# astra-vision/PaSCo

Hardware: AMD Instinct MI355X
Metric: scenes/sec (256x256x32, ~10% occ) PaSCo MIMO-3 (higher is better)
Workload: dtype f32 (conv products as 3 x f16 split MFMA, fp32 accumulate)

## Files before the change

pasco_amd/csrc/conv_grid.hip:

```cpp
#include <math.h>
#include <stdlib.h>

#include "conv_h2_common.h"

constexpr int GR_WROWS = 264;
constexpr int GR_PIECES = GR_WROWS / 8;
constexpr int GR_ROUNDS = (GR_PIECES + 7) / 8;
constexpr int GR_WIN = GR_WROWS * 128;
constexpr int GR_BST = 128 * 128;
constexpr int GR_OFF_WIN = 2 * GR_BST;
constexpr int GR_OFF_ZERO = GR_OFF_WIN + 2 * GR_WIN;
constexpr int GR_OFF_MISC = GR_OFF_ZERO + 128;
constexpr int GR_LDS = GR_OFF_MISC + 64;

template <bool EMIT>
__global__ void __launch_bounds__(512, 2) k_conv_grid(ConvArgsH a) {
  constexpr int WN = 2, TM = 2, TN = 2;
  constexpr int NT = 512;
  constexpr int BM = 256, BN = 128;
  constexpr int NMH = TM * TN * 3;
  constexpr int NRH = (TM + TN) * 2;
  __shared__ __attribute__((aligned(128))) char lds[GR_LDS];

  int tile = blockIdx.x;
  if (PH_ABLATE(a, 0x200)) tile = ((int)blockIdx.x & 7) * ((int)gridDim.x >> 3) + ((int)blockIdx.x >> 3);
  if (tile >= a.n_row_tiles * a.n_col_tiles) return;
  const int row_tile = tile / a.n_col_tiles;
  const int col_tile = tile - row_tile * a.n_col_tiles;
  const int64_t m0 = (int64_t)row_tile * BM;
  const int n0 = col_tile * BN;

  const int tid = threadIdx.x;
  const int lane = tid & 63;
  const int wave = __builtin_amdgcn_readfirstlane(tid >> 6);
  const int wm = wave / WN, wn = wave % WN;
  const int h = lane >> 5;
  const int l31 = lane & 31;

  const int GX = a.gdim[1], GY = a.gdim[2], GZ = a.gdim[3];
  const int kx = a.gker[0], ky = a.gker[1], kz = a.gker[2];
  const int hx = kx >> 1, hy = ky >> 1, hz = kz >> 1;
  const int ngroups = kx * kz;
  const int cout = a.cout;
  const int nchunks = a.cpad >> 5;
  const uint32_t rsb = 4u * (uint32_t)a.cpad;
  const int slice = (int)blockIdx.y;

  f32x16 acc[TM][TN];
#pragma unroll
  for (int i = 0; i < TM; ++i)
#pragma unroll
    for (int j = 0; j < TN; ++j)
#pragma unroll
      for (int r = 0; r < 16; ++r) acc[i][j][r] = 0.f;

  unsigned *gmask = reinterpret_cast<unsigned *>(lds + GR_OFF_MISC);
  if (tid < 2) gmask[tid] = 0u;
  if (tid < 32) reinterpret_cast<float *>(lds + GR_OFF_ZERO)[tid] = 0.f;
  __syncthreads();
  {
    const int r = tid & 255;
    const int64_t s = m0 + r;
    const bool ok = s < a.n_out;
    const int t = (int)((ok ? s : 0) / GY);
    const int x = t % GX, zz = (t / GX) % GZ;
    for (int g = tid >> 8; g < ngroups; g += 2) {
      const int ix = g % kx, iz = g / kx;
      const bool v = ok && (unsigned)(x + ix - hx) < (unsigned)GX && (unsigned)(zz + iz - hz) < (unsigned)GZ;
      if (__ballot(v) != 0ull && lane == 0) atomicOr(&gmask[g >> 5], 1u << (g & 31));
    }
  }
  __syncthreads();
  const unsigned long long gm =
      (unsigned long long)(unsigned)__builtin_amdgcn_readfirstlane(gmask[0]) |
      ((unsigned long long)(unsigned)__builtin_amdgcn_readfirstlane(gmask[1]) << 32);
  const int nvalid = __builtin_popcountll(gm);
  const int total_units = nvalid * nchunks;
  int nsl = a.ksplit;
  if (a.grid_upw > 0) {
    nsl = (total_units + (a.grid_upw >> 1)) / a.grid_upw;
    nsl = nsl < 1 ? 1 : (nsl > a.ksplit ? a.ksplit : nsl);
  }
  const int nunits = (slice < nsl && slice < total_units) ? (total_units - slice + nsl - 1) / nsl : 0;
  const int nstages = nunits * ky;

  if (nstages > 0) {
    struct Unit {
      int n, vi, g, c;
    };
    const int kq = nsl / nchunks, kr = nsl - kq * nchunks;
    const int inv_kx = 65536 / kx + 1;
    auto first_unit = [&]() {
      Unit u;
      u.n = 0;
      u.vi = slice / nchunks;
      u.c = slice - u.vi * nchunks;
      unsigned long long m = gm;
      for (int q = 0; q < u.vi; ++q) m &= m - 1;
      u.g = __builtin_ctzll(m);
      return u;
    };
    auto next_unit = [&](const Unit &p) {
      Unit u;
      u.n = p.n + 1;
      u.c = p.c + kr;
      u.vi = p.vi + kq;
      if (u.c >= nchunks) {
        u.c -= nchunks;
        ++u.vi;
      }
      unsigned long long m = gm & ~((2ull << p.g) - 1ull);
      int g = p.g;
      for (int q = p.vi; q < u.vi; ++q) {
        g = __builtin_ctzll(m);
        m &= m - 1;
      }
      u.g = g;
      return u;
    };

    const int l_j = tid & 7;
    const int l_r = tid >> 3;
    const uint32_t sj16 = (uint32_t)((l_j ^ ((l_r >> 1) & 7)) << 4);
    const uint64_t w_base = (uint64_t)reinterpret_cast<uintptr_t>(a.w_split) + sj16;
    uint32_t boff[2];
#pragma unroll
    for (int q = 0; q < 2; ++q) {
      int n = n0 + l_r + q * 64;
      n = n < cout ? n : cout - 1;
      boff[q] = (uint32_t)n * rsb;
    }
    const int64_t wslab = (int64_t)cout * rsb;
    const uint64_t in_base = (uint64_t)reinterpret_cast<uintptr_t>(a.in_split);
    const int wl_r = lane >> 3;
    const int n_last = (int)(a.n_in - 1);
    const uint32_t wdst0 = (uint32_t)(wave * 1024);
    const uint32_t bdst0 = (uint32_t)(wave * 1024);

    auto fire_b = [&](uint64_t src, char *bbuf, int q) {
      if (PH_ABLATE(a, 2)) return;
      char *dst = bbuf + bdst0 + q * 8192;
      __builtin_amdgcn_global_load_lds((const __attribute__((address_space(1))) void *)(uintptr_t)(src + boff[q]),
                                       (__attribute__((address_space(3))) void *)dst, 16, 0, 0);
    };
    auto fire_win = [&](int first, uint32_t coff, uint32_t wbuf, int round) {
      if (PH_ABLATE(a, 1)) return;
      const int R = round * 64 + wave * 8 + wl_r;
      int site = first + R;
      site = site < 0 ? 0 : (site > n_last ? n_last : site);
      const uint64_t src = in_base + (uint64_t)(uint32_t)site * rsb + coff + (uint32_t)((l_j ^ ((R >> 1) & 7)) << 4);
      char *dst = lds + wbuf + round * 8192 + wdst0;
      __builtin_amdgcn_global_load_lds((const __attribute__((address_space(1))) void *)(uintptr_t)src,
                                       (__attribute__((address_space(3))) void *)dst, 16, 0, 0);
    };
    struct WinSrc {
      int first;
      uint32_t coff, wbuf;
    };
    auto win_of = [&](const Unit &u) {
      const int iz = (u.g * inv_kx) >> 16, ix = u.g - iz * kx;
      WinSrc w;
      w.first = (int)m0 + (ix - hx) * GY + (iz - hz) * GX * GY - hy;
      w.coff = (uint32_t)u.c << 7;
      w.wbuf = (uint32_t)(GR_OFF_WIN + (u.n & 1) * GR_WIN);
      return w;
    };

    int ay[TM], ax[TM], az[TM];
    bool aok[TM];
    uint32_t rbase[TM];
#pragma unroll
    for (int i = 0; i < TM; ++i) {
      rbase[i] = (uint32_t)(wm * 64 + i * 32 + l31);
      const int64_t s = m0 + rbase[i];
      aok[i] = s < a.n_out;
      const int sc = aok[i] ? (int)s : 0;
      const int t = sc / GY;
      ay[i] = sc - t * GY;
      ax[i] = t % GX;
      az[i] = (t / GX) % GZ;
    }
    const uint32_t hq = (uint32_t)h << 4;
    struct ASet {
      uint32_t row[TM], sw[TM];
    };
    bool gv[TM];
    uint32_t cwb = 0;
    auto unit_valid = [&](const Unit &u) {
      const int iz = (u.g * inv_kx) >> 16, ix = u.g - iz * kx;
      cwb = (uint32_t)(GR_OFF_WIN + (u.n & 1) * GR_WIN);
#pragma unroll
      for (int i = 0; i < TM; ++i)
        gv[i] = aok[i] && (unsigned)(ax[i] + ix - hx) < (unsigned)GX && (unsigned)(az[i] + iz - hz) < (unsigned)GZ;
    };
    auto a_set = [&](int iy, ASet &s) {
#pragma unroll
      for (int i = 0; i < TM; ++i) {
        const uint32_t R = rbase[i] + (uint32_t)iy;
        const bool v = gv[i] && (unsigned)(ay[i] + iy - hy) < (unsigned)GY;
        s.row[i] = v ? cwb + R * 128u : (uint32_t)GR_OFF_ZERO;
        s.sw[i] = ((R >> 1) & 7u) << 4;
      }
    };

    const int sw = (l31 >> 1) & 7;
    uint32_t xo[2][2];
#pragma unroll
    for (int ks = 0; ks < 2; ++ks)
#pragma unroll
      for (int part = 0; part < 2; ++part) xo[ks][part] = (uint32_t)(((part * 4 + ks * 2 + h) ^ sw) << 4);
    const uint32_t brow = (uint32_t)((wn * TN * 32 + l31) * 128);
    struct Frag {
      f16x8 ah[2][TM], al[2][TM], bh[2][TN], bl[2][TN];
    };
    Frag f;
    ASet aset;
    auto read_one = [&](const char *bbuf, int ks, int r) {
      if (PH_ABLATE(a, 8)) return;
      if (r < 2 * TM) {
        const int i = r >> 1, part = r & 1;
        const uint32_t o = aset.row[i] + ((((uint32_t)(part * 4 + ks * 2) << 4) | hq) ^ aset.sw[i]);
        if (part == 0) f.ah[ks][i] = *reinterpret_cast<const f16x8 *>(lds + o);
        else f.al[ks][i] = *reinterpret_cast<const f16x8 *>(lds + o);
      } else {
        const int j = (r - 2 * TM) >> 1;
        if (((r - 2 * TM) & 1) == 0) f.bh[ks][j] = *reinterpret_cast<const f16x8 *>(bbuf + brow + j * 4096 + xo[ks][0]);
        else f.bl[ks][j] = *reinterpret_cast<const f16x8 *>(bbuf + brow + j * 4096 + xo[ks][1]);
      }
    };
    auto mfma_one = [&](int ks, int m) {
      if (PH_ABLATE(a, 4)) return;
      const int ij = m % (TM * TN), p = m / (TM * TN);
      const int i = ij / TN, j = ij % TN;
      if (p == 0) acc[i][j] = __builtin_amdgcn_mfma_f32_32x32x16_f16(f.bh[ks][j], f.al[ks][i], acc[i][j], 0, 0, 0);
      else if (p == 1) acc[i][j] = __builtin_amdgcn_mfma_f32_32x32x16_f16(f.bl[ks][j], f.ah[ks][i], acc[i][j], 0, 0, 0);
      else acc[i][j] = __builtin_amdgcn_mfma_f32_32x32x16_f16(f.bh[ks][j], f.ah[ks][i], acc[i][j], 0, 0, 0);
    };

    Unit cu = first_unit(), du = cu;
    int ciy = 0, diy = 0;
    bool nu_ok = nunits > 1;
    Unit nu = nu_ok ? next_unit(cu) : cu;
    WinSrc nw = win_of(nu);
    uint64_t wsrc = w_base + (uint64_t)((int64_t)(ky * du.g) * wslab) + ((uint32_t)du.c << 7);
    auto d_step = [&]() {
      if (du.n == nunits - 1 && diy == ky - 1) return;
      if (++diy == ky) {
        diy = 0;
        du = next_unit(du);
        wsrc = w_base + (uint64_t)((int64_t)(ky * du.g) * wslab) + ((uint32_t)du.c << 7);
      } else {
        wsrc += (uint64_t)wslab;
      }
    };
    const int rps = (GR_ROUNDS + ky - 2) / (ky - 1);

    char *b0 = lds, *b1 = lds + GR_BST;
    {
      const WinSrc w0 = win_of(cu);
      for (int q = 0; q < GR_ROUNDS; ++q)
        if (q * 8 + wave < GR_PIECES) fire_win(w0.first, w0.coff, w0.wbuf, q);
    }
    fire_b(wsrc, b0, 0);
    fire_b(wsrc, b0, 1);
    d_step();
    fire_b(wsrc, b1, 0);
    fire_b(wsrc, b1, 1);
    d_step();
    unit_valid(cu);
    a_set(0, aset);
    asm volatile("s_waitcnt vmcnt(0) lgkmcnt(0)" ::: "memory");
    __builtin_amdgcn_s_barrier();
#pragma unroll
    for (int r = 0; r < NRH; ++r) read_one(b0, 0, r);
    asm volatile("s_waitcnt lgkmcnt(0)" ::: "memory");

    auto half_a = [&](const char *cur) {
#pragma unroll
      for (int g = 0; g < NRH; ++g) {
        read_one(cur, 1, g);
        __builtin_amdgcn_sched_barrier(0);
#pragma unroll
        for (int m = g * NMH / NRH; m < (g + 1) * NMH / NRH; ++m) mfma_one(0, m);
        __builtin_amdgcn_sched_barrier(0);
      }
    };
    auto half_b = [&](char *cur, const char *nxt) {
      int wq = (nu_ok && ciy < ky - 1) ? ciy * rps : GR_ROUNDS;
      const int wq_end = wq + rps;
      const WinSrc w = nw;
      if (!(cu.n == nunits - 1 && ciy == ky - 1)) {
        if (++ciy == ky) {
          ciy = 0;
          cu = nu;
          nu_ok = cu.n + 1 < nunits;
          if (nu_ok) {
            nu = next_unit(cu);
            nw = win_of(nu);
          }
          unit_valid(cu);
        }
      }
      if (!PH_ABLATE(a, 64)) a_set(ciy, aset);
#pragma unroll
      for (int g = 0; g < NRH; ++g) {
        if (g < 2) fire_b(wsrc, cur, g);
        if (g >= 2 && g < 5) {
          if (wq < wq_end && wq * 8 + wave < GR_PIECES) fire_win(w.first, w.coff, w.wbuf, wq);
          ++wq;
        }
        read_one(nxt, 0, g);
        if (g == 5) d_step();
        __builtin_amdgcn_sched_barrier(0);
#pragma unroll
        for (int m = g * NMH / NRH; m < (g + 1) * NMH / NRH; ++m) mfma_one(1, m);
        __builtin_amdgcn_sched_barrier(0);
      }
    };
#define GRID_MIDDLE()                                                            \
  do {                                                                           \
    if (PH_ABLATE(a, 16)) asm volatile("s_waitcnt lgkmcnt(0)" ::: "memory");     \
    else asm volatile("s_waitcnt vmcnt(0) lgkmcnt(0)" ::: "memory");             \
    if (!PH_ABLATE(a, 32)) __builtin_amdgcn_s_barrier();                         \
  } while (0)
    for (int s = 0; s < nstages; s += 2) {
      half_a(b0);
      GRID_MIDDLE();
      half_b(b0, b1);
      asm volatile("s_waitcnt lgkmcnt(0)" ::: "memory");
      if (s + 1 >= nstages) break;
      half_a(b1);
      GRID_MIDDLE();
      half_b(b1, b0);
      asm volatile("s_waitcnt lgkmcnt(0)" ::: "memory");
    }
    asm volatile("s_waitcnt vmcnt(0)" ::: "memory");
#undef GRID_MIDDLE
  }

  h2_store_tile<TM, TN, EMIT>(a, acc, m0, n0, wm, wn, h, l31);
}

#ifdef PH_DEV
static int g_grid_ablate = 0;
extern "C" void ph_conv_grid_set_ablate(int mask) { g_grid_ablate = mask; }
#else
constexpr int g_grid_ablate = 0;
#endif

static double grid_groups(const int *gd, const int *gk) {
  double zavg = 0.0;
  for (int z = 0; z < gd[3]; ++z)
    for (int iz = 0; iz < gk[2]; ++iz) zavg += (z + iz - gk[2] / 2 >= 0 && z + iz - gk[2] / 2 < gd[3]) ? 1.0 : 0.0;
  return gk[0] * zavg / gd[3];
}

int ph_conv_grid_try(const ConvArgsH &a_in, hipStream_t st) {
  const int *gd = a_in.gdim, *gk = a_in.gker;
  if (gd[0] <= 0 || a_in.tile_k != nullptr || a_in.win_gather || (a_in.cpad & 31) || a_in.cout % 128 != 0 || a_in.in_split == nullptr ||
      a_in.axis_table != nullptr)
    return -1;
  if (a_in.route & PH_ROUTE_GRID_NEVER) return -1;
  const int kx = gk[0], ky = gk[1], kz = gk[2];
  if (ky < 3 || ky > 7 || !(kx & 1) || !(ky & 1) || !(kz & 1) || kx * kz > 64 || kx * ky * kz != a_in.kvol) return -1;
  const int64_t sites = (int64_t)gd[0] * gd[1] * gd[2] * gd[3];
  if (sites != a_in.n_out || sites != a_in.n_in || gd[2] < 1) return -1;
  ConvArgsH a = a_in;
  a.n_row_tiles = (int)((a.n_out + 255) / 256);
  a.n_col_tiles = a.cout / 128;
  const int64_t tiles = (int64_t)a.n_row_tiles * a.n_col_tiles;
  const int nchunks = a.cpad >> 5;
  const double units = grid_groups(gd, gk) * nchunks;
  const double stage_us = 1.0, fixed_us = 8.0;
  int best = 1;
  double best_us = 1e30;
  for (int ks = 1; ks <= 12; ++ks) {
    if (ks > 1 && (a.tail_ws == nullptr || a.tail_ws_bytes < (int64_t)ks * a.n_out * a.cout * 4)) break;
    if (ks > 1 && units / ks < 2.0) break;
    const double rounds = (double)((tiles * ks + 255) / 256);
    double us = rounds * (ceil(units / ks) * ky * stage_us + fixed_us);
    if (ks > 1) us += (double)ks * (double)a.n_out * a.cout * 4.0 / 3.0e6 + 5.0;
    if (us < best_us) best_us = us, best = ks;
  }
  if (const char *e = PH_DEV_ENV("PASCO_GRID_KS")) {
    const int ks = atoi(e);
    if (ks >= 1 && (ks == 1 || (a.tail_ws != nullptr && a.tail_ws_bytes >= (int64_t)ks * a.n_out * a.cout * 4))) best = ks;
  }
  a.grid_upw = 0;
  if (best > 1 && tiles * best <= 256) {
    const int upw = (int)(units / best + 0.5) > 0 ? (int)(units / best + 0.5) : 1;
    int zmax = 0;
    for (int z = 0; z < gd[3]; ++z) {
      int c = 0;
      for (int iz = 0; iz < kz; ++iz) c += (z + iz - kz / 2 >= 0 && z + iz - kz / 2 < gd[3]) ? 1 : 0;
      zmax = c > zmax ? c : zmax;
    }
    const int zreach = zmax + 1 < kz ? zmax + 1 : kz;
    int ksmax = (kx * zreach * nchunks + upw / 2) / upw;
    ksmax = ksmax > 12 ? 12 : ksmax;
    while (ksmax > best && a.tail_ws_bytes < (int64_t)ksmax * a.n_out * a.cout * 4) --ksmax;
    const char *e = PH_DEV_ENV("PASCO_GRID_UPW");
    if (e == nullptr || atoi(e) != 0) {
      if (ksmax > best) best = ksmax;
      a.grid_upw = upw;
    }
  }
  a.ksplit = best;
  a.partial = best > 1 ? (float *)a.tail_ws : nullptr;
  a.win_stats = nullptr;
  a.ablate = g_grid_ablate;
  const int grid = (int)((tiles + 7) / 8) * 8;
  const bool emit = a.out_split != nullptr && a.ksplit == 1;
  if (emit) hipLaunchKernelGGL((k_conv_grid<true>), dim3(grid, 1), dim3(512), 0, st, a);
  else hipLaunchKernelGGL((k_conv_grid<false>), dim3(grid, a.ksplit), dim3(512), 0, st, a);
  PH_LAUNCH_CHECK();
  if (a.ksplit > 1) {
    if (int rc = ph_launch_splitk_epilogue(a, st)) return rc;
  }
  ph_record_cfg(2, 256, 128, 32, a.ksplit, emit ? 1 : 0, 8, 8);
  return 0;
}
```

pasco_amd/me/backend.py:

```python
from __future__ import annotations

import contextlib
import ctypes as C
import os
import threading
from typing import Dict, Optional

import torch

from .._clib import _raw_stream, bind

_HERE = os.path.dirname(os.path.abspath(__file__))
HIP_LIB_PATH = os.path.join(os.path.dirname(_HERE), "csrc", "libpascohip.so")

ACT_NONE, ACT_RELU, ACT_LEAKY = 0, 1, 2
ABI_VERSION = 5


class StatusError(RuntimeError):

    def __init__(self, bits: int, message: str):
        super().__init__(message)
        self.bits = bits

# ... 383 lines not shown
                        raise ValueError(f"conv: {name} has {t.numel()} entries, expected {cout}")
            d.out_split, d.osp_scale, d.osp_shift, d.osp_act = _ptr(out_split), _ptr(osc), _ptr(osh), int(oact)
        d.in_, d.weight, d.nbr, d.out = (None if x.is_meta else _ptr(x)), _ptr(weight), _ptr(nbr), _ptr(out)
        d.n_in, d.n_out, d.cin, d.cout, d.kvol = x.shape[0], n_out, cin, cout, kvol
        d.pro_act, d.epi_act, d.res_act, d.epi_slope = pro_act, epi_act, res_act, float(slope)
        for name, t, c in (("pro_scale", pro_scale, cin), ("pro_shift", pro_shift, cin),
                           ("bias", bias, cout), ("epi_scale", epi_scale, cout),
                           ("epi_shift", epi_shift, cout), ("epi2_scale", epi2_scale, cout),
                           ("epi2_shift", epi2_shift, cout)):
            if t is not None:
                self._chk(t, torch.float32, name)
                if t.numel() != c:
                    raise ValueError(f"conv: {name} has {t.numel()} entries, expected {c}")
            setattr(d, name, _ptr(t))
        if residual is not None:
            self._chk(residual, torch.float32, "residual")
            if tuple(residual.shape) != (n_out, cout):
                raise ValueError("conv: residual shape mismatch")
        d.residual = _ptr(residual)
        if axis is not None:
            tab, acoords, lo = axis
            self._chk(tab, torch.float32, "axis table")
            self._chk(acoords, torch.int32, "axis coords")
            if tab.dim() != 3 or tab.shape[0] != 3 or tab.shape[2] != cout or tuple(acoords.shape) != (n_out, 4):
                raise ValueError("conv: axis = (table [3, T, cout], coords [n_out, 4], lo)")
            if self.device_type == "cuda" and (split is None or len(split) != 2):
                raise ValueError("conv: the axis-table residual is served by the pre-split (mode 2) path")
            d.axis_table, d.axis_coords, d.axis_lo, d.axis_rows = _ptr(tab), _ptr(acoords), int(lo), int(tab.shape[1])
        if split is not None:
            if len(split) == 2:
                w_split, unscale = split
                if in_split is None:
                    in_split = self.split_rows(x, pro_scale=pro_scale, pro_shift=pro_shift, pro_act=pro_act, slope=slope)
                elif not x.is_meta and (pro_scale is not None or pro_shift is not None or pro_act != ACT_NONE) and \
                        not in_split_has_prologue:
                    raise ValueError("conv: in_split given together with a prologue - pass in_split_has_prologue=True if "
                                     "the operand was built with split_rows(x, pro_scale=..., pro_shift=..., pro_act=...), "
                                     "else drop in_split")
                cpad = (cin + 31) // 32 * 32
                if in_split.dtype != torch.float16 or in_split.numel() != x.shape[0] * 2 * cpad:
                    raise ValueError("conv: in_split does not match the input rows")
                if w_split.numel() != kvol * cout * 2 * cpad:
                    raise ValueError("conv: w_split does not match the kernel")
                d.mma_mode, d.in_split, d.w_split = 2, _ptr(in_split), _ptr(w_split)
                if grid is not None and nbr is not None:
                    gd, gk = grid
                    if len(gd) != 4 or len(gk) != 3 or gd[0] * gd[1] * gd[2] * gd[3] != n_out or x.shape[0] != n_out or \
                            gk[0] * gk[1] * gk[2] != kvol or any(k % 2 == 0 for k in gk):
                        raise ValueError("conv: grid = ((B, X, Y, Z), (kx, ky, kz)) must describe the whole map (odd kernel sizes)")
                    for q in range(4):
                        d.grid_dims[q] = int(gd[q])
                    for q in range(3):
                        d.grid_kernel[q] = int(gk[q])
                if rowlist is not None and nbr is not None:
                    d.rl_in, d.rl_out, d.rl_tile_k = _ptr(rowlist["in"]), _ptr(rowlist["out"]), _ptr(rowlist["tile_k"])
                    d.rl_rows, d.rl_tiles = int(rowlist["in"].numel()), int(rowlist["tile_k"].numel())
                if win is not None and kvol == 27 and nbr is not None:
                    d.win_rows, d.win_cnt, d.win_slots, d.win_stats = (_ptr(win["rows"]), _ptr(win["cnt"]),
                                                                       _ptr(win["slots"]), _ptr(win["stats"]))
                    if 32 < cout <= 64 and self._serves_cuda:
                        d.w_frag = _ptr(self.weight_fragments(w_split, kvol, cout, cpad))
            else:
                w_hi, w_lo, unscale = split
                d.mma_mode, d.w_f16_hi, d.w_f16_lo = 1, _ptr(w_hi), _ptr(w_lo)
            d.split_exp2 = SPLIT_ACT_EXP2
            d.w_unscale = float(unscale) * 2.0 ** (-SPLIT_ACT_EXP2)
            d.status = self.status_ptr(dev) if status is None else status.data_ptr()
            if kvol > 1 or n_out * cout <= (1 << 23):
                need = 12 * n_out * cout * 4 if n_out * cout <= (1 << 23) else 512 * 128 * 128 * 4
                key = ("splitk",) + self._stream_key(dev)
                sk = self._ws.get(key)
                if sk is None or sk.numel() < need:
                    sk = torch.empty(need, dtype=torch.uint8, device=dev)
                    self._ws[key] = sk
                d.splitk_ws, d.splitk_ws_bytes = _ptr(sk), sk.numel()
        if exact_if is not None:
            if split is not None:
                raise ValueError("conv: exact_if guards an exact fp32 launch (no split)")
            d.exact_if = exact_if.data_ptr()
        rc = self.fn["conv_fwd"](C.byref(d), self.stream(dev))
        self._check(rc, "conv_fwd")
        return (out, out_split) if emit else out

    @staticmethod
    def grid_offsets(kernel_size) -> list:
        kx, ky, kz = (int(k) for k in kernel_size)
        return [(x, y, z) for z in range(-(kz // 2), kz // 2 + 1) for x in range(-(kx // 2), kx // 2 + 1)
                for y in range(-(ky // 2), ky // 2 + 1)]

    def conv_last_config(self) -> dict:
        buf = (_i32 * 8)()
        self._check(self.fn["conv_last_config"](C.cast(buf, _vp)), "conv_last_config")
        names = ("mma_mode", "bm", "bn", "kc", "ksplit", "emit", "kernel", "waves")
        return dict(zip(names, [int(v) for v in buf]))

    def status_word(self, device) -> torch.Tensor:
        return self._status_pair(device)[0:1]

    def status_ptr(self, device) -> int:
        pinned = getattr(self._tls, "status_pin", None)
        if pinned is not None:
            return pinned.data_ptr()
        idx = device.index
        if idx is None and device.type == "cuda":
            idx = torch.cuda.current_device()
        k = (device.type, idx, _raw_stream(idx) if device.type == "cuda" else 0)
# ... 66 lines not shown
        w = weight.detach().float()
        if w.dim() == 2:
            w = w[None]
        if exponent is not None:
            e = int(exponent)
        else:
            wmax = float(w.abs().max())
            e = 0 if wmax == 0.0 else 13 - int(torch.frexp(torch.tensor(wmax))[1])
        scaled = (w * float(2.0 ** e)).transpose(1, 2).contiguous()
        hi = scaled.to(torch.float16)
        lo = (scaled - hi.float()).to(torch.float16)
        return hi.contiguous(), lo.contiguous(), float(2.0 ** (-e))

    def split_rows(self, x: torch.Tensor, *, pro_scale=None, pro_shift=None, pro_act=ACT_NONE, slope=0.01,
                   out: Optional[torch.Tensor] = None, exp2: Optional[int] = None,
                   status: Optional[torch.Tensor] = None) -> torch.Tensor:
        exp2 = SPLIT_ACT_EXP2 if exp2 is None else int(exp2)
        self._chk(x, torch.float32, "in")
        n, c = x.shape
        if c % 8 != 0:
            raise ValueError("split_rows: needs c % 8 == 0")
        cpad = (c + 31) // 32 * 32
        if out is None:
            out = torch.empty((n, cpad // 32, 2, 32), dtype=torch.float16, device=x.device)
        for name, t in (("pro_scale", pro_scale), ("pro_shift", pro_shift)):
            if t is not None:
                self._chk(t, torch.float32, name)
                if t.numel() != c:
                    raise ValueError(f"split_rows: {name} has {t.numel()} entries, expected {c}")
        rc = self.fn["split_rows"](_ptr(x), n, c, _ptr(pro_scale), _ptr(pro_shift), pro_act, float(slope), exp2, _ptr(out),
                                   self.status_ptr(x.device) if status is None else status.data_ptr(), self.stream(x.device))
        self._check(rc, "split_rows")
        return out

    def split_weight_rows(self, weight: torch.Tensor, exponent=None):
        w = weight.detach().float()
        if w.dim() == 2:
            w = w[None]
        if exponent is not None:
            e = int(exponent)
        else:
            wmax = float(w.abs().max())
            e = 0 if wmax == 0.0 else 13 - int(torch.frexp(torch.tensor(wmax))[1])
        k, cin, cout = w.shape
        rows = (w * float(2.0 ** e)).transpose(1, 2).contiguous().view(k * cout, cin)
        return self.split_rows(rows, exp2=0), float(2.0 ** (-e))

    @staticmethod
    def weight_fragments(w_split: torch.Tensor, kvol: int, cout: int, cpad: int) -> torch.Tensor:
        hit = getattr(w_split, "_ph_wfrag", None)
        if hit is not None and hit[0] == (kvol, cout, cpad):
            return hit[1]
        g = cpad // 32
        ws = w_split.view(kvol, cout, g, 2, 2, 2, 8)
        rows = torch.arange(64, device=w_split.device).clamp_(max=cout - 1)
        ws = ws.index_select(1, rows).view(kvol, 2, 32, g, 2, 2, 2, 8)
        frag = ws.permute(0, 3, 5, 1, 4, 6, 2, 7).contiguous()
        frag = frag.view(kvol, 2 * g, 2, 2, 64, 8)
        try:
            w_split._ph_wfrag = ((kvol, cout, cpad), frag)
        except AttributeError:
            pass
        return frag

    def split_capable(self) -> bool:
        return self.device_type == "cuda" or self.checker_split

    def split_supported(self, cin: int, cout: int) -> bool:
        return self.split_capable() and cin % 8 == 0 and cout % 4 == 0

    def maxpool_fwd(self, x: torch.Tensor, nbr: torch.Tensor) -> torch.Tensor:
        self._chk(x, torch.float32, "in")
        self._chk(nbr, torch.int32, "nbr")
        kvol, n_out = nbr.shape
        out = torch.empty((n_out, x.shape[1]), dtype=torch.float32, device=x.device)
        rc = self.fn["maxpool_fwd"](_ptr(x), x.shape[1], _ptr(nbr), kvol, n_out, _ptr(out),
                                    self.stream(x.device))
        self._check(rc, "maxpool_fwd")
        return out

    def mask_compact(self, mask: torch.Tensor) -> torch.Tensor:
        if mask.dtype == torch.bool:
            mask = mask.view(torch.uint8)
        self._chk(mask, torch.uint8, "mask")
        n = mask.shape[0]
        dev = mask.device
        buf = torch.empty(max(n, 1) + 1, dtype=torch.int32, device=dev)
        keep, cnt = buf[:-1], buf[-1:]
        ws = self.workspace(n, dev)
        rc = self.fn["mask_compact"](_ptr(mask), n, _ptr(keep), cnt.data_ptr(), _ptr(ws), ws.numel(),
                                     self.stream(dev))
        self._check(rc, "mask_compact")
        return keep[: int(cnt.item())]

    MAX_INPUT_SITES = 1 << 27

    def pooled_merge(self, h: torch.Tensor, xyz: torch.Tensor, starts, bounds=None):
        self._chk(h, torch.float32, "h")
        self._chk(xyz, torch.int64, "xyz")
        n, c = h.shape
        m = len(starts) - 1
        if not (c % 4 == 0 and 1 <= m <= 8 and tuple(xyz.shape) == (n, 3)):
            raise ValueError("pooled_merge: h [P, C] with C % 4 == 0, xyz int64 [P, 3], at most 8 subnets")
        dev = h.device
        st = self.stream(dev)
        if bounds is None:
            b6 = torch.empty(6, dtype=torch.int32, device=dev)
            self._check(self.fn["points_bounds"](_ptr(xyz), n, _ptr(b6), st), "points_bounds")
            b6 = b6.tolist()
            lo, hi = b6[:3], b6[3:]
        else:
# ... 431 lines not shown
```

Baseline: 47.01.

## Load grid-conv weights from prearranged fragments into registers, drop LDS weight staging

The grid convolution kernel stops staging weight tiles in LDS. Each wave now loads prearranged MFMA weight fragments straight from global memory into registers with inline-asm loads, and the workgroup shrinks from 512 to 256 threads, each wave covering four row tiles. The window buffer is resized and the MFMA, LDS-read and weight-load schedule is hand-interleaved with sched barriers. The host split-K planner is replaced by a cached cost model that uses per-row-tile group counts, and the Python backend builds the fragment layout for any multiple-of-64 output width. The risks are higher register pressure, dependence on hand-placed waitcnt counts being correct, and the global weight loads adding latency.

```diff
diff --git a/pasco_amd/csrc/conv_grid.hip b/pasco_amd/csrc/conv_grid.hip
--- a/pasco_amd/csrc/conv_grid.hip
+++ b/pasco_amd/csrc/conv_grid.hip
@@ -3,27 +3,40 @@
 
 #include "conv_h2_common.h"
 
-constexpr int GR_WROWS = 264;
-constexpr int GR_PIECES = GR_WROWS / 8;
-constexpr int GR_ROUNDS = (GR_PIECES + 7) / 8;
+constexpr int GR_ROUNDS = 9;
+constexpr int GR_WROWS = GR_ROUNDS * 32;
 constexpr int GR_WIN = GR_WROWS * 128;
-constexpr int GR_BST = 128 * 128;
-constexpr int GR_OFF_WIN = 2 * GR_BST;
-constexpr int GR_OFF_ZERO = GR_OFF_WIN + 2 * GR_WIN;
+constexpr int GR_OFF_ZERO = 2 * GR_WIN;
 constexpr int GR_OFF_MISC = GR_OFF_ZERO + 128;
 constexpr int GR_LDS = GR_OFF_MISC + 64;
+static_assert(2 * GR_LDS <= 160 * 1024, "two workgroups per CU");
+static_assert(GR_WROWS >= 256 + 7 - 1, "a window holds the run of a ky = 7 group");
+
+struct GrW {
+  f16x8 bh[2], bl[2];
+};
+struct GrA {
+  f16x8 h[2], l[2];
+};
+#define GR_PIN_W(w) "+v"((w).bh[0]), "+v"((w).bh[1]), "+v"((w).bl[0]), "+v"((w).bl[1])
+#define GR_PIN_A(f) "+v"((f).h[0]), "+v"((f).h[1]), "+v"((f).l[0]), "+v"((f).l[1])
+#define GR_SB() __builtin_amdgcn_sched_barrier(0)
+#define GR_GLD(dst, voff, base, OFFS) \
+  asm volatile("global_load_dwordx4 %0, %1, %2 offset:" #OFFS : "=v"(dst) : "v"(voff), "s"(base) : "memory")
+
+__device__ __forceinline__ f16x8 gr_lds(uint32_t addr) {
+  f16x8 v;
+  asm volatile("ds_read_b128 %0, %1" : "=v"(v) : "v"(addr) : "memory");
+  return v;
+}
 
 template <bool EMIT>
-__global__ void __launch_bounds__(512, 2) k_conv_grid(ConvArgsH a) {
-  constexpr int WN = 2, TM = 2, TN = 2;
-  constexpr int NT = 512;
+__global__ void __launch_bounds__(256, 2) k_conv_grid(ConvArgsH a) {
+  constexpr int TM = 4, TN = 2;
   constexpr int BM = 256, BN = 128;
-  constexpr int NMH = TM * TN * 3;
-  constexpr int NRH = (TM + TN) * 2;
   __shared__ __attribute__((aligned(128))) char lds[GR_LDS];
 
-  int tile = blockIdx.x;
-  if (PH_ABLATE(a, 0x200)) tile = ((int)blockIdx.x & 7) * ((int)gridDim.x >> 3) + ((int)blockIdx.x >> 3);
+  const int tile = blockIdx.x;
   if (tile >= a.n_row_tiles * a.n_col_tiles) return;
   const int row_tile = tile / a.n_col_tiles;
   const int col_tile = tile - row_tile * a.n_col_tiles;
@@ -33,7 +46,7 @@
   const int tid = threadIdx.x;
   const int lane = tid & 63;
   const int wave = __builtin_amdgcn_readfirstlane(tid >> 6);
-  const int wm = wave / WN, wn = wave % WN;
+  const int wm = wave >> 1, wn = wave & 1;
   const int h = lane >> 5;
   const int l31 = lane & 31;
 
@@ -41,10 +54,16 @@
   const int kx = a.gker[0], ky = a.gker[1], kz = a.gker[2];
   const int hx = kx >> 1, hy = ky >> 1, hz = kz >> 1;
   const int ngroups = kx * kz;
-  const int cout = a.cout;
   const int nchunks = a.cpad >> 5;
   const uint32_t rsb = 4u * (uint32_t)a.cpad;
   const int slice = (int)blockIdx.y;
+#ifdef PH_DEV
+  int abl_bits = a.ablate;
+  asm volatile("" : "+s"(abl_bits));
+#define GR_ABL(bits) (abl_bits & (bits))
+#else
+#define GR_ABL(bits) 0
+#endif
 
   f32x16 acc[TM][TN];
 #pragma unroll
@@ -59,13 +78,13 @@
   if (tid < 32) reinterpret_cast<float *>(lds + GR_OFF_ZERO)[tid] = 0.f;
   __syncthreads();
   {
-    const int r = tid & 255;
-    const int64_t s = m0 + r;
+    const int64_t s = m0 + tid;
     const bool ok = s < a.n_out;
     const int t = (int)((ok ? s : 0) / GY);
     const int x = t % GX, zz = (t / GX) % GZ;
-    for (int g = tid >> 8; g < ngroups; g += 2) {
-      const int ix = g % kx, iz = g / kx;
+    const int inv = 65536 / kx + 1;
+    for (int g = 0; g < ngroups; ++g) {
+      const int iz = (g * inv) >> 16, ix = g - iz * kx;
       const bool v = ok && (unsigned)(x + ix - hx) < (unsigned)GX && (unsigned)(zz + iz - hz) < (unsigned)GZ;
       if (__ballot(v) != 0ull && lane == 0) atomicOr(&gmask[g >> 5], 1u << (g & 31));
     }
@@ -82,9 +101,8 @@
     nsl = nsl < 1 ? 1 : (nsl > a.ksplit ? a.ksplit : nsl);
   }
   const int nunits = (slice < nsl && slice < total_units) ? (total_units - slice + nsl - 1) / nsl : 0;
-  const int nstages = nunits * ky;
-
-  if (nstages > 0) {
+
+  if (nunits > 0) {
     struct Unit {
       int n, vi, g, c;
     };
@@ -119,224 +137,192 @@
       return u;
     };
 
-    const int l_j = tid & 7;
-    const int l_r = tid >> 3;
-    const uint32_t sj16 = (uint32_t)((l_j ^ ((l_r >> 1) & 7)) << 4);
-    const uint64_t w_base = (uint64_t)reinterpret_cast<uintptr_t>(a.w_split) + sj16;
-    uint32_t boff[2];
-#pragma unroll
-    for (int q = 0; q < 2; ++q) {
-      int n = n0 + l_r + q * 64;
-      n = n < cout ? n : cout - 1;
-      boff[q] = (uint32_t)n * rsb;
-    }
-    const int64_t wslab = (int64_t)cout * rsb;
-    const uint64_t in_base = (uint64_t)reinterpret_cast<uintptr_t>(a.in_split);
+    const uint32_t lds0 = (uint32_t)(uintptr_t)(__attribute__((address_space(3))) char *)lds;
+    const int l_j = lane & 7;
     const int wl_r = lane >> 3;
     const int n_last = (int)(a.n_in - 1);
-    const uint32_t wdst0 = (uint32_t)(wave * 1024);
-    const uint32_t bdst0 = (uint32_t)(wave * 1024);
-
-    auto fire_b = [&](uint64_t src, char *bbuf, int q) {
-      if (PH_ABLATE(a, 2)) return;
-      char *dst = bbuf + bdst0 + q * 8192;
-      __builtin_amdgcn_global_load_lds((const __attribute__((address_space(1))) void *)(uintptr_t)(src + boff[q]),
-                                       (__attribute__((address_space(3))) void *)dst, 16, 0, 0);
-    };
-    auto fire_win = [&](int first, uint32_t coff, uint32_t wbuf, int round) {
-      if (PH_ABLATE(a, 1)) return;
-      const int R = round * 64 + wave * 8 + wl_r;
-      int site = first + R;
+    const int wrow0 = wave * 8 + wl_r;
+    const uint64_t in_base = (uint64_t)reinterpret_cast<uintptr_t>(a.in_split) + (uint32_t)((l_j ^ ((wrow0 >> 1) & 7)) << 4);
+    auto fire_win = [&](int first, uint32_t coff, int wbuf, int round) {
+      if (GR_ABL(1)) return;
+      int site = first + round * 32 + wrow0;
       site = site < 0 ? 0 : (site > n_last ? n_last : site);
-      const uint64_t src = in_base + (uint64_t)(uint32_t)site * rsb + coff + (uint32_t)((l_j ^ ((R >> 1) & 7)) << 4);
-      char *dst = lds + wbuf + round * 8192 + wdst0;
+      const uint64_t src = in_base + (uint64_t)(uint32_t)site * rsb + coff;
+      char *dst = lds + wbuf + round * 4096 + wave * 1024;
       __builtin_amdgcn_global_load_lds((const __attribute__((address_space(1))) void *)(uintptr_t)src,
                                        (__attribute__((address_space(3))) void *)dst, 16, 0, 0);
     };
     struct WinSrc {
-      int first;
-      uint32_t coff, wbuf;
+      int first, wbuf;
+      uint32_t coff;
     };
     auto win_of = [&](const Unit &u) {
       const int iz = (u.g * inv_kx) >> 16, ix = u.g - iz * kx;
       WinSrc w;
       w.first = (int)m0 + (ix - hx) * GY + (iz - hz) * GX * GY - hy;
       w.coff = (uint32_t)u.c << 7;
-      w.wbuf = (uint32_t)(GR_OFF_WIN + (u.n & 1) * GR_WIN);
+      w.wbuf = (u.n & 1) * GR_WIN;
       return w;
     };
 
+    const int nch16 = a.cpad >> 4;
+    const int ncg = a.cout >> 6;
+    const uint64_t cstride = (uint64_t)ncg << 12;
+    const uint64_t kstride = cstride * (uint64_t)nch16;
+    const uint64_t wbase = (uint64_t)reinterpret_cast<uintptr_t>(a.w_frag) + (uint64_t)(((n0 >> 6) + wn) << 12);
+    const uint32_t wlane = (uint32_t)lane * 16u;
+    auto w_unit = [&](const Unit &u) -> uint64_t {
+      return wbase + (uint64_t)(ky * u.g) * kstride + (uint64_t)(2 * u.c) * cstride;
+    };
+
+    const int rbase0 = wm * 128 + l31;
     int ay[TM], ax[TM], az[TM];
-    bool aok[TM];
-    uint32_t rbase[TM];
 #pragma unroll
     for (int i = 0; i < TM; ++i) {
-      rbase[i] = (uint32_t)(wm * 64 + i * 32 + l31);
-      const int64_t s = m0 + rbase[i];
-      aok[i] = s < a.n_out;
-      const int sc = aok[i] ? (int)s : 0;
+      const int64_t s = m0 + rbase0 + 32 * i;
+      const bool ok = s < a.n_out;
+      const int sc = ok ? (int)s : 0;
       const int t = sc / GY;
-      ay[i] = sc - t * GY;
-      ax[i] = t % GX;
-      az[i] = (t / GX) % GZ;
+      ay[i] = sc - t * GY - hy;
+      ax[i] = ok ? t % GX - hx : -(1 << 20);
+      az[i] = (t / GX) % GZ - hz;
     }
     const uint32_t hq = (uint32_t)h << 4;
-    struct ASet {
-      uint32_t row[TM], sw[TM];
-    };
-    bool gv[TM];
-    uint32_t cwb = 0;
+    const uint32_t zaddr = lds0 + (uint32_t)GR_OFF_ZERO;
+    int ayu[TM];
+    uint32_t cwb = lds0;
+    uint32_t ad[TM];
     auto unit_valid = [&](const Unit &u) {
       const int iz = (u.g * inv_kx) >> 16, ix = u.g - iz * kx;
-      cwb = (uint32_t)(GR_OFF_WIN + (u.n & 1) * GR_WIN);
+      cwb = lds0 + (uint32_t)((u.n & 1) * GR_WIN);
 #pragma unroll
       for (int i = 0; i < TM; ++i)
-        gv[i] = aok[i] && (unsigned)(ax[i] + ix - hx) < (unsigned)GX && (unsigned)(az[i] + iz - hz) < (unsigned)GZ;
-    };
-    auto a_set = [&](int iy, ASet &s) {
-#pragma unroll
-      for (int i = 0; i < TM; ++i) {
-        const uint32_t R = rbase[i] + (uint32_t)iy;
-        const bool v = gv[i] && (unsigned)(ay[i] + iy - hy) < (unsigned)GY;
-        s.row[i] = v ? cwb + R * 128u : (uint32_t)GR_OFF_ZERO;
-        s.sw[i] = ((R >> 1) & 7u) << 4;
-      }
-    };
-
-    const int sw = (l31 >> 1) & 7;
-    uint32_t xo[2][2];
-#pragma unroll
-    for (int ks = 0; ks < 2; ++ks)
-#pragma unroll
-      for (int part = 0; part < 2; ++part) xo[ks][part] = (uint32_t)(((part * 4 + ks * 2 + h) ^ sw) << 4);
-    const uint32_t brow = (uint32_t)((wn * TN * 32 + l31) * 128);
-    struct Frag {
-      f16x8 ah[2][TM], al[2][TM], bh[2][TN], bl[2][TN];
-    };
-    Frag f;
-    ASet aset;
-    auto read_one = [&](const char *bbuf, int ks, int r) {
-      if (PH_ABLATE(a, 8)) return;
-      if (r < 2 * TM) {
-        const int i = r >> 1, part = r & 1;
-        const uint32_t o = aset.row[i] + ((((uint32_t)(part * 4 + ks * 2) << 4) | hq) ^ aset.sw[i]);
-        if (part == 0) f.ah[ks][i] = *reinterpret_cast<const f16x8 *>(lds + o);
-        else f.al[ks][i] = *reinterpret_cast<const f16x8 *>(lds + o);
-      } else {
-        const int j = (r - 2 * TM) >> 1;
-        if (((r - 2 * TM) & 1) == 0) f.bh[ks][j] = *reinterpret_cast<const f16x8 *>(bbuf + brow + j * 4096 + xo[ks][0]);
-        else f.bl[ks][j] = *reinterpret_cast<const f16x8 *>(bbuf + brow + j * 4096 + xo[ks][1]);
-      }
-    };
-    auto mfma_one = [&](int ks, int m) {
-      if (PH_ABLATE(a, 4)) return;
-      const int ij = m % (TM * TN), p = m / (TM * TN);
-      const int i = ij / TN, j = ij % TN;
-      if (p == 0) acc[i][j] = __builtin_amdgcn_mfma_f32_32x32x16_f16(f.bh[ks][j], f.al[ks][i], acc[i][j], 0, 0, 0);
-      else if (p == 1) acc[i][j] = __builtin_amdgcn_mfma_f32_32x32x16_f16(f.bl[ks][j], f.ah[ks][i], acc[i][j], 0, 0, 0);
-      else acc[i][j] = __builtin_amdgcn_mfma_f32_32x32x16_f16(f.bh[ks][j], f.ah[ks][i], acc[i][j], 0, 0, 0);
-    };
-
-    Unit cu = first_unit(), du = cu;
-    int ciy = 0, diy = 0;
+        ayu[i] = ((unsigned)(ax[i] + ix) < (unsigned)GX && (unsigned)(az[i] + iz) < (unsigned)GZ) ? ay[i] : -(1 << 20);
+    };
+    auto a_addr = [&](int iy, int i) {
+      const uint32_t R = (uint32_t)(rbase0 + 32 * i + iy);
+      const bool v = (unsigned)(ayu[i] + iy) < (unsigned)GY && iy < ky;
+      const uint32_t row = v ? cwb + R * 128u : zaddr;
+      ad[i] = row + (hq ^ (((R >> 1) & 7u) << 4));
+    };
+
+    GrW w0, w1;
+    GrA fa, fb;
+    auto mf = [&](const GrW &w, const GrA &f, int i0, int n) {
+      if (GR_ABL(4)) return;
+      const int p = n >> 2, u = (n >> 1) & 1, j = n & 1;
+      if (p == 0) acc[i0 + u][j] = __builtin_amdgcn_mfma_f32_32x32x16_f16(w.bh[j], f.l[u], acc[i0 + u][j], 0, 0, 0);
+      else if (p == 1) acc[i0 + u][j] = __builtin_amdgcn_mfma_f32_32x32x16_f16(w.bl[j], f.h[u], acc[i0 + u][j], 0, 0, 0);
+      else acc[i0 + u][j] = __builtin_amdgcn_mfma_f32_32x32x16_f16(w.bh[j], f.h[u], acc[i0 + u][j], 0, 0, 0);
+    };
+    auto read_a = [&](GrA &f, int i0, uint32_t c) {
+      if (GR_ABL(8)) return;
+      f.h[0] = gr_lds(ad[i0] ^ c);
+      f.l[0] = gr_lds(ad[i0] ^ (c | 64u));
+      f.h[1] = gr_lds(ad[i0 + 1] ^ c);
+      f.l[1] = gr_lds(ad[i0 + 1] ^ (c | 64u));
+    };
+    auto load_w = [&](GrW &w, uint64_t p, int q) {
+      if (GR_ABL(2)) return;
+      if (q == 0) GR_GLD(w.bh[0], wlane, p, 0);
+      else if (q == 1) GR_GLD(w.bl[0], wlane, p, 1024);
+      else if (q == 2) GR_GLD(w.bh[1], wlane, p, 2048);
+      else GR_GLD(w.bl[1], wlane, p, 3072);
+    };
+
+    Unit cu = first_unit();
     bool nu_ok = nunits > 1;
     Unit nu = nu_ok ? next_unit(cu) : cu;
     WinSrc nw = win_of(nu);
-    uint64_t wsrc = w_base + (uint64_t)((int64_t)(ky * du.g) * wslab) + ((uint32_t)du.c << 7);
-    auto d_step = [&]() {
-      if (du.n == nunits - 1 && diy == ky - 1) return;
-      if (++diy == ky) {
-        diy = 0;
-        du = next_unit(du);
-        wsrc = w_base + (uint64_t)((int64_t)(ky * du.g) * wslab) + ((uint32_t)du.c << 7);
-      } else {
-        wsrc += (uint64_t)wslab;
-      }
-    };
-    const int rps = (GR_ROUNDS + ky - 2) / (ky - 1);
-
-    char *b0 = lds, *b1 = lds + GR_BST;
+    int wq = 0, wq_end = nu_ok ? GR_ROUNDS : 0;
+    const bool two = ky < 5;
+
+    auto step = [&](auto ks_tag, GrW &wc, GrW &wx, uint64_t wpn, int iyn) {
+      constexpr int KS = decltype(ks_tag)::value;
+      constexpr uint32_t CN = KS == 0 ? 32u : 0u;
+      asm volatile("s_waitcnt lgkmcnt(4)" : GR_PIN_A(fa)::"memory");
+      asm volatile("s_waitcnt vmcnt(0)" : GR_PIN_W(wc)::"memory");
+      GR_SB(); mf(wc, fa, 0, 0); GR_SB();
+      if (wq < wq_end) {
+        fire_win(nw.first, nw.coff, nw.wbuf, wq);
+        ++wq;
+      }
+      GR_SB(); mf(wc, fa, 0, 1); GR_SB();
+      if (two && wq < wq_end) {
+        fire_win(nw.first, nw.coff, nw.wbuf, wq);
+        ++wq;
+      }
+      GR_SB(); mf(wc, fa, 0, 2); GR_SB();
+      load_w(wx, wpn, 0);
+      GR_SB(); mf(wc, fa, 0, 3); GR_SB();
+      load_w(wx, wpn, 1);
+      GR_SB(); mf(wc, fa, 0, 4); GR_SB();
+      load_w(wx, wpn, 2);
+      GR_SB(); mf(wc, fa, 0, 5); GR_SB();
+      load_w(wx, wpn, 3);
+      GR_SB(); mf(wc, fa, 0, 6); GR_SB();
+      if (KS == 1) a_addr(iyn, 0);
+      GR_SB(); mf(wc, fa, 0, 7); GR_SB();
+      if (KS == 1) a_addr(iyn, 1);
+      GR_SB(); mf(wc, fa, 0, 8); GR_SB();
+      if (KS == 1) a_addr(iyn, 2);
+      GR_SB(); mf(wc, fa, 0, 9); GR_SB();
+      if (KS == 1) a_addr(iyn, 3);
+      GR_SB(); mf(wc, fa, 0, 10); GR_SB(); mf(wc, fa, 0, 11); GR_SB();
+      read_a(fa, 0, CN);
+      asm volatile("s_waitcnt lgkmcnt(4)" : GR_PIN_A(fb)::"memory");
+      if (GR_ABL(8)) asm volatile("s_waitcnt lgkmcnt(0)" ::: "memory");
+      GR_SB(); mf(wc, fb, 2, 0); GR_SB(); mf(wc, fb, 2, 1); GR_SB(); mf(wc, fb, 2, 2); GR_SB(); mf(wc, fb, 2, 3); GR_SB();
+      mf(wc, fb, 2, 4); GR_SB(); mf(wc, fb, 2, 5); GR_SB(); mf(wc, fb, 2, 6); GR_SB(); mf(wc, fb, 2, 7); GR_SB();
+      mf(wc, fb, 2, 8); GR_SB(); mf(wc, fb, 2, 9); GR_SB(); mf(wc, fb, 2, 10); GR_SB(); mf(wc, fb, 2, 11); GR_SB();
+      read_a(fb, 2, CN);
+      GR_SB();
+    };
+
     {
-      const WinSrc w0 = win_of(cu);
-      for (int q = 0; q < GR_ROUNDS; ++q)
-        if (q * 8 + wave < GR_PIECES) fire_win(w0.first, w0.coff, w0.wbuf, q);
-    }
-    fire_b(wsrc, b0, 0);
-    fire_b(wsrc, b0, 1);
-    d_step();
-    fire_b(wsrc, b1, 0);
-    fire_b(wsrc, b1, 1);
-    d_step();
-    unit_valid(cu);
-    a_set(0, aset);
-    asm volatile("s_waitcnt vmcnt(0) lgkmcnt(0)" ::: "memory");
+      const WinSrc wf = win_of(cu);
+#pragma unroll
+      for (int q = 0; q < GR_ROUNDS; ++q) fire_win(wf.first, wf.coff, wf.wbuf, q);
+    }
+    uint64_t wp = w_unit(cu);
+#pragma unroll
+    for (int q = 0; q < 4; ++q) load_w(w0, wp, q);
+    asm volatile("s_waitcnt vmcnt(0) lgkmcnt(0)" : GR_PIN_W(w0)::"memory");
     __builtin_amdgcn_s_barrier();
-#pragma unroll
-    for (int r = 0; r < NRH; ++r) read_one(b0, 0, r);
-    asm volatile("s_waitcnt lgkmcnt(0)" ::: "memory");
-
-    auto half_a = [&](const char *cur) {
-#pragma unroll
-      for (int g = 0; g < NRH; ++g) {
-        read_one(cur, 1, g);
-        __builtin_amdgcn_sched_barrier(0);
-#pragma unroll
-        for (int m = g * NMH / NRH; m < (g + 1) * NMH / NRH; ++m) mfma_one(0, m);
-        __builtin_amdgcn_sched_barrier(0);
-      }
-    };
-    auto half_b = [&](char *cur, const char *nxt) {
-      int wq = (nu_ok && ciy < ky - 1) ? ciy * rps : GR_ROUNDS;
-      const int wq_end = wq + rps;
-      const WinSrc w = nw;
-      if (!(cu.n == nunits - 1 && ciy == ky - 1)) {
-        if (++ciy == ky) {
-          ciy = 0;
-          cu = nu;
-          nu_ok = cu.n + 1 < nunits;
-          if (nu_ok) {
-            nu = next_unit(cu);
-            nw = win_of(nu);
-          }
-          unit_valid(cu);
-        }
-      }
-      if (!PH_ABLATE(a, 64)) a_set(ciy, aset);
-#pragma unroll
-      for (int g = 0; g < NRH; ++g) {
-        if (g < 2) fire_b(wsrc, cur, g);
-        if (g >= 2 && g < 5) {
-          if (wq < wq_end && wq * 8 + wave < GR_PIECES) fire_win(w.first, w.coff, w.wbuf, wq);
-          ++wq;
-        }
-        read_one(nxt, 0, g);
-        if (g == 5) d_step();
-        __builtin_amdgcn_sched_barrier(0);
-#pragma unroll
-        for (int m = g * NMH / NRH; m < (g + 1) * NMH / NRH; ++m) mfma_one(1, m);
-        __builtin_amdgcn_sched_barrier(0);
-      }
-    };
-#define GRID_MIDDLE()                                                            \
-  do {                                                                           \
-    if (PH_ABLATE(a, 16)) asm volatile("s_waitcnt lgkmcnt(0)" ::: "memory");     \
-    else asm volatile("s_waitcnt vmcnt(0) lgkmcnt(0)" ::: "memory");             \
-    if (!PH_ABLATE(a, 32)) __builtin_amdgcn_s_barrier();                         \
-  } while (0)
-    for (int s = 0; s < nstages; s += 2) {
-      half_a(b0);
-      GRID_MIDDLE();
-      half_b(b0, b1);
-      asm volatile("s_waitcnt lgkmcnt(0)" ::: "memory");
-      if (s + 1 >= nstages) break;
-      half_a(b1);
-      GRID_MIDDLE();
-      half_b(b1, b0);
-      asm volatile("s_waitcnt lgkmcnt(0)" ::: "memory");
-    }
-    asm volatile("s_waitcnt vmcnt(0)" ::: "memory");
-#undef GRID_MIDDLE
-  }
+
+    for (int n = 0; n < nunits; ++n) {
+      unit_valid(cu);
+#pragma unroll
+      for (int i = 0; i < TM; ++i) a_addr(0, i);
+      GR_SB();
+      read_a(fa, 0, 0u);
+      read_a(fb, 2, 0u);
+      GR_SB();
+      const uint64_t wpu = nu_ok ? w_unit(nu) : wp;
+      uint64_t wk = wp;
+      int iy_last = ky - 1;
+      asm volatile("" : "+s"(iy_last));
+#pragma clang loop unroll(disable)
+      for (int iy = 0; iy < ky; ++iy) {
+        step(std::integral_constant<int, 0>(), w0, w1, wk + cstride, iy);
+        const uint64_t wkn = iy < iy_last ? wk + kstride : wpu;
+        step(std::integral_constant<int, 1>(), w1, w0, wkn, iy + 1);
+        wk = wkn;
+      }
+      asm volatile("s_waitcnt vmcnt(0) lgkmcnt(0)" : GR_PIN_W(w0), GR_PIN_A(fa), GR_PIN_A(fb)::"memory");
+      __builtin_amdgcn_s_barrier();
+      wp = wpu;
+      cu = nu;
+      nu_ok = cu.n + 1 < nunits;
+      if (nu_ok) {
+        nu = next_unit(cu);
+        nw = win_of(nu);
+      }
+      wq = 0;
+      wq_end = nu_ok ? GR_ROUNDS : 0;
+    }
+  }
+#undef GR_ABL
 
   h2_store_tile<TM, TN, EMIT>(a, acc, m0, n0, wm, wn, h, l31);
 }
@@ -354,11 +340,104 @@
     for (int iz = 0; iz < gk[2]; ++iz) zavg += (z + iz - gk[2] / 2 >= 0 && z + iz - gk[2] / 2 < gd[3]) ? 1.0 : 0.0;
   return gk[0] * zavg / gd[3];
 }
+static int grid_tile_groups(const int *gd, const int *gk, int64_t row_tile, int64_t n_out) {
+  const int GX = gd[1], GY = gd[2], GZ = gd[3], kx = gk[0], kz = gk[2];
+  const int64_t s0 = row_tile * 256, s1 = (s0 + 255 < n_out ? s0 + 255 : n_out - 1);
+  unsigned long long mask = 0ull;
+  const unsigned long long full = kx * kz >= 64 ? ~0ull : (1ull << (kx * kz)) - 1ull;
+  for (int64_t t = s0 / GY; t <= s1 / GY && mask != full; ++t) {
+    const int x = (int)(t % GX), z = (int)((t / GX) % GZ);
+    for (int iz = 0; iz < kz; ++iz) {
+      if (z + iz - kz / 2 < 0 || z + iz - kz / 2 >= GZ) continue;
+      for (int ix = 0; ix < kx; ++ix)
+        if (x + ix - kx / 2 >= 0 && x + ix - kx / 2 < GX) mask |= 1ull << (iz * kx + ix);
+    }
+  }
+  return __builtin_popcountll(mask);
+}
+
+struct GridPlan {
+  int key[10];
+  int ksplit, upw;
+};
+static void grid_plan(const ConvArgsH &a, int64_t tiles, int *ksplit, int *upw_out) {
+  const int *gd = a.gdim, *gk = a.gker;
+  const int nchunks = a.cpad >> 5, ky = gk[1];
+  const double slab = (double)a.n_out * a.cout * 4.0;
+  int cap = 1;
+  if (a.tail_ws != nullptr && slab > 0.0) {
+    const int64_t fit = a.tail_ws_bytes / ((int64_t)a.n_out * a.cout * 4);
+    cap = fit > 11 ? 11 : (fit < 1 ? 1 : (int)fit);
+  }
+  thread_local GridPlan cache[8];
+  thread_local int cache_n = 0, cache_at = 0;
+  GridPlan pl{};
+  const int key[10] = {gd[0], gd[1], gd[2], gd[3], gk[0], gk[1], gk[2], a.cpad, a.cout, cap};
+  for (int q = 0; q < 10; ++q) pl.key[q] = key[q];
+  for (int i = 0; i < cache_n; ++i) {
+    bool same = true;
+    for (int q = 0; q < 10; ++q) same &= cache[i].key[q] == key[q];
+    if (same) {
+      *ksplit = cache[i].ksplit, *upw_out = cache[i].upw;
+      return;
+    }
+  }
+  const double stage_alone_us = 1.35, stage_pair_us = 2.0, fixed_us = 8.0;
+  const int resident = 512;
+  auto cost = [&](int maxper, int64_t wgs, int ks) {
+    double us;
+    if (wgs <= resident) us = maxper * ky * (wgs <= 256 ? stage_alone_us : stage_pair_us) + fixed_us;
+    else us = (double)((wgs + resident - 1) / resident) * (maxper * ky * stage_pair_us + fixed_us);
+    if (ks > 1) us += ks * slab / 3.0e6 + 5.0;
+    return us;
+  };
+  const double units = grid_groups(gd, gk) * nchunks;
+  const int ct = a.n_col_tiles, nrt = a.n_row_tiles;
+  int *tu = tiles <= resident / 2 ? (int *)malloc(sizeof(int) * (size_t)nrt) : nullptr;
+  int tu_max = (int)ceil(units);
+  if (tu != nullptr) {
+    tu_max = 0;
+    for (int r = 0; r < nrt; ++r) {
+      tu[r] = grid_tile_groups(gd, gk, r, a.n_out) * nchunks;
+      tu_max = tu[r] > tu_max ? tu[r] : tu_max;
+    }
+  }
+  int best = 1, best_upw = 0;
+  double best_us = 1e30;
+  for (int ks = 1; ks <= cap; ++ks) {
+    if (ks > 1 && units / ks < 2.0) break;
+    const double us = cost((tu_max + ks - 1) / ks, tiles * ks, ks);
+    if (us < best_us) best_us = us, best = ks, best_upw = 0;
+  }
+  if (cap > 1 && tu != nullptr) {
+    for (int upw = tu_max; upw >= 2; --upw) {
+      int64_t wgs = 0;
+      int ksl = 0, maxper = 0;
+      for (int r = 0; r < nrt; ++r) {
+        int nsl = (tu[r] + (upw >> 1)) / upw;
+        nsl = nsl < 1 ? 1 : (nsl > cap ? cap : nsl);
+        const int per = (tu[r] + nsl - 1) / nsl;
+        wgs += (int64_t)nsl * ct;
+        ksl = nsl > ksl ? nsl : ksl;
+        maxper = per > maxper ? per : maxper;
+      }
+      if (wgs > resident - 16 || ksl < 2) continue;
+      const double us = cost(maxper, wgs, ksl);
+      if (us < best_us) best_us = us, best = ksl, best_upw = upw;
+    }
+  }
+  free(tu);
+  pl.ksplit = best, pl.upw = best_upw;
+  cache[cache_at] = pl;
+  cache_at = (cache_at + 1) & 7;
+  cache_n = cache_n < 8 ? cache_n + 1 : 8;
+  *ksplit = best, *upw_out = best_upw;
+}
 
 int ph_conv_grid_try(const ConvArgsH &a_in, hipStream_t st) {
   const int *gd = a_in.gdim, *gk = a_in.gker;
   if (gd[0] <= 0 || a_in.tile_k != nullptr || a_in.win_gather || (a_in.cpad & 31) || a_in.cout % 128 != 0 || a_in.in_split == nullptr ||
-      a_in.axis_table != nullptr)
+      a_in.axis_table != nullptr || a_in.w_frag == nullptr)
     return -1;
   if (a_in.route & PH_ROUTE_GRID_NEVER) return -1;
   const int kx = gk[0], ky = gk[1], kz = gk[2];
@@ -369,54 +448,29 @@
   a.n_row_tiles = (int)((a.n_out + 255) / 256);
   a.n_col_tiles = a.cout / 128;
   const int64_t tiles = (int64_t)a.n_row_tiles * a.n_col_tiles;
-  const int nchunks = a.cpad >> 5;
-  const double units = grid_groups(gd, gk) * nchunks;
-  const double stage_us = 1.0, fixed_us = 8.0;
-  int best = 1;
-  double best_us = 1e30;
-  for (int ks = 1; ks <= 12; ++ks) {
-    if (ks > 1 && (a.tail_ws == nullptr || a.tail_ws_bytes < (int64_t)ks * a.n_out * a.cout * 4)) break;
-    if (ks > 1 && units / ks < 2.0) break;
-    const double rounds = (double)((tiles * ks + 255) / 256);
-    double us = rounds * (ceil(units / ks) * ky * stage_us + fixed_us);
-    if (ks > 1) us += (double)ks * (double)a.n_out * a.cout * 4.0 / 3.0e6 + 5.0;
-    if (us < best_us) best_us = us, best = ks;
-  }
+  int best = 1, upw = 0;
+  grid_plan(a, tiles, &best, &upw);
+  const int64_t slab = (int64_t)a.n_out * a.cout * 4;
   if (const char *e = PH_DEV_ENV("PASCO_GRID_KS")) {
     const int ks = atoi(e);
-    if (ks >= 1 && (ks == 1 || (a.tail_ws != nullptr && a.tail_ws_bytes >= (int64_t)ks * a.n_out * a.cout * 4))) best = ks;
-  }
-  a.grid_upw = 0;
-  if (best > 1 && tiles * best <= 256) {
-    const int upw = (int)(units / best + 0.5) > 0 ? (int)(units / best + 0.5) : 1;
-    int zmax = 0;
-    for (int z = 0; z < gd[3]; ++z) {
-      int c = 0;
-      for (int iz = 0; iz < kz; ++iz) c += (z + iz - kz / 2 >= 0 && z + iz - kz / 2 < gd[3]) ? 1 : 0;
-      zmax = c > zmax ? c : zmax;
-    }
-    const int zreach = zmax + 1 < kz ? zmax + 1 : kz;
-    int ksmax = (kx * zreach * nchunks + upw / 2) / upw;
-    ksmax = ksmax > 12 ? 12 : ksmax;
-    while (ksmax > best && a.tail_ws_bytes < (int64_t)ksmax * a.n_out * a.cout * 4) --ksmax;
-    const char *e = PH_DEV_ENV("PASCO_GRID_UPW");
-    if (e == nullptr || atoi(e) != 0) {
-      if (ksmax > best) best = ksmax;
-      a.grid_upw = upw;
-    }
-  }
+    if (ks >= 1 && (ks == 1 || (a.tail_ws != nullptr && a.tail_ws_bytes >= ks * slab))) best = ks, upw = 0;
+  }
+  if (const char *e = PH_DEV_ENV("PASCO_GRID_UPW")) {
+    upw = atoi(e) > 0 ? atoi(e) : 0;
+  }
+  a.grid_upw = best > 1 ? upw : 0;
   a.ksplit = best;
   a.partial = best > 1 ? (float *)a.tail_ws : nullptr;
   a.win_stats = nullptr;
   a.ablate = g_grid_ablate;
-  const int grid = (int)((tiles + 7) / 8) * 8;
+  const int grid = (int)tiles;
   const bool emit = a.out_split != nullptr && a.ksplit == 1;
-  if (emit) hipLaunchKernelGGL((k_conv_grid<true>), dim3(grid, 1), dim3(512), 0, st, a);
-  else hipLaunchKernelGGL((k_conv_grid<false>), dim3(grid, a.ksplit), dim3(512), 0, st, a);
+  if (emit) hipLaunchKernelGGL((k_conv_grid<true>), dim3(grid, 1), dim3(256), 0, st, a);
+  else hipLaunchKernelGGL((k_conv_grid<false>), dim3(grid, a.ksplit), dim3(256), 0, st, a);
   PH_LAUNCH_CHECK();
   if (a.ksplit > 1) {
     if (int rc = ph_launch_splitk_epilogue(a, st)) return rc;
   }
-  ph_record_cfg(2, 256, 128, 32, a.ksplit, emit ? 1 : 0, 8, 8);
+  ph_record_cfg(2, 256, 128, 32, a.ksplit, emit ? 1 : 0, 8, 4);
   return 0;
 }
diff --git a/pasco_amd/me/backend.py b/pasco_amd/me/backend.py
--- a/pasco_amd/me/backend.py
+++ b/pasco_amd/me/backend.py
@@ -459,6 +459,8 @@
                         d.grid_dims[q] = int(gd[q])
                     for q in range(3):
                         d.grid_kernel[q] = int(gk[q])
+                    if cout % 128 == 0 and self._serves_cuda:
+                        d.w_frag = _ptr(self.weight_fragments(w_split, kvol, cout, cpad))
                 if rowlist is not None and nbr is not None:
                     d.rl_in, d.rl_out, d.rl_tile_k = _ptr(rowlist["in"]), _ptr(rowlist["out"]), _ptr(rowlist["tile_k"])
                     d.rl_rows, d.rl_tiles = int(rowlist["in"].numel()), int(rowlist["tile_k"].numel())
@@ -631,11 +633,12 @@
         if hit is not None and hit[0] == (kvol, cout, cpad):
             return hit[1]
         g = cpad // 32
+        m = (cout + 63) // 64
         ws = w_split.view(kvol, cout, g, 2, 2, 2, 8)
-        rows = torch.arange(64, device=w_split.device).clamp_(max=cout - 1)
-        ws = ws.index_select(1, rows).view(kvol, 2, 32, g, 2, 2, 2, 8)
-        frag = ws.permute(0, 3, 5, 1, 4, 6, 2, 7).contiguous()
-        frag = frag.view(kvol, 2 * g, 2, 2, 64, 8)
+        rows = torch.arange(64 * m, device=w_split.device).clamp_(max=cout - 1)
+        ws = ws.index_select(1, rows).view(kvol, m, 2, 32, g, 2, 2, 2, 8)
+        frag = ws.permute(0, 4, 6, 1, 2, 5, 7, 3, 8).contiguous()
+        frag = frag.view(kvol, 2 * g, 2, 2, 64, 8) if m == 1 else frag.view(kvol, 2 * g, m, 2, 2, 64, 8)
         try:
             w_split._ph_wfrag = ((kvol, cout, cpad), frag)
         except AttributeError:
```

After: 45.92. 0.977x the previous value.
